# AlphacatPlus/VmambaIR

Hardware: AMD Instinct MI355X
Metric: images/sec, x4 SR 64->256 training step (fwd+bwd+Adam+EMA), full VmambaIR UNet (higher is better)
Workload: dtype bf16; 1 GPU; BASELINE.json configs[1]: x4 SR 64x64 LQ, MambaSISR6 dim48 [15,1,1,1]+15, bf16 autocast (scan arithmetic f32), batch 8 per GPU; global_batch=8, per_gpu_batch=8, parallelism=dp1, step_launch=hipGraph replay, vendor_conv_solver_search=True, vendor_conv_solver_records=bench_data/miopen, optimizer=Adam 2e-4 (0.9,0.99) + EMA 0.999, loss=L1, rccl_ranks=1, allreduce_overlapped=False, allreduce_buckets=1, allreduce_bytes=0

## Files before the change

### include/vmambair_oss.h

```cpp
#ifndef VMAMBAIR_OSS_H
#define VMAMBAIR_OSS_H

#include <stddef.h>
#include <stdint.h>

#ifdef __cplusplus
extern "C" {
#endif

#define OSS_OK 0
#define OSS_ERR_NULL (-1)
#define OSS_ERR_SHAPE (-2)
#define OSS_ERR_DSTATE (-3)
#define OSS_ERR_WORKSPACE (-4)

#define OSS_MAX_DSTATE 256

typedef enum {
    OSS_F32 = 0, OSS_F16 = 1, OSS_BF16 = 2,
    OSS_F32_BF16X3 = 3
} oss_dtype;

typedef void *oss_stream_t;

// ... 162 lines not shown
    float *zt;
    float *dts;
    float *hs;
    float *y;
    float *yc;
    float *stat;
    float *c;
    const float *pool_part;
    int n_part;
    float pool_scale;
} oss_chan_params;
int oss_chan_fwd(const oss_chan_params *p, oss_stream_t stream);
size_t oss_chan_grad_floats(int L, int dc, int Rc, int Cc);
size_t oss_chan_bwd_scratch_floats(int B, int L, int dc, int Rc, int Cc);
int oss_chan_bwd(const oss_chan_params *p, const float *gc, float *dpooled, float *grads, float *scratch, oss_stream_t stream);
int oss_rowsum(oss_dtype io, const void *a, const void *bmul, float *out, int batch, int channels, int pixels,
               int64_t a_batch_stride, int64_t a_channel_stride, int64_t b_batch_stride, int64_t b_channel_stride, float alpha,
               oss_stream_t stream);
int oss_row_affine(oss_dtype io, const void *x, const float *mul, const float *add, void *y, int batch, int channels,
                   int pixels, int64_t x_batch_stride, int64_t x_channel_stride, float alpha, oss_stream_t stream);

int oss_gelu_gate_fwd(oss_dtype io, const void *h, void *out, int batch, size_t half_elems, int64_t h_batch_stride,
                      oss_stream_t stream);
int oss_gelu_gate_bwd(oss_dtype io, const void *h, const void *dout, void *dh, int batch, size_t half_elems,
                      int64_t h_batch_stride, int64_t dout_batch_stride, oss_stream_t stream);

typedef struct {
    const void *src;
    void *dst;
    int64_t stride;
// ... 118 lines not shown
```

### vmambair_amd/csrc/oss_capi.hip

```cpp
#include <atomic>
#include <cstdlib>
#include <mutex>
#include <vector>
#include <cstring>
#include <algorithm>
#include "oss_device.h"
#include "oss_host.h"

namespace oss {

static std::atomic<int> g_force_fwd{-1}, g_force_bwd{-1};
static std::atomic<int> g_last_fwd{-1}, g_last_bwd{-1};
static std::atomic<int> g_force_fwd_seg{-1}, g_force_bwd_seg{-1};
std::atomic<int> g_last_fwd_segments{1}, g_last_bwd_segments{1}, g_last_bwd_lane_states{0};

int scan_pick_segments(long wgs, int n_chunks, int seg_req, double ovh) {
    if (seg_req == 0 || seg_req == 1 || n_chunks < 2 || wgs <= 0) return 1;
    if (seg_req > 1) return std::min(std::min(seg_req, n_chunks), kMaxSegments);
    if (wgs >= 256) return 1;
    int best = 1;
    double best_cost = (double)n_chunks;
    for (int s = 2; s <= std::min(n_chunks, 16); ++s) {
        const int cps = (n_chunks + s - 1) / s;
        if ((n_chunks + cps - 1) / cps != s) continue;
// ... 564 lines not shown
int oss_chan_fwd(const oss_chan_params *p, oss_stream_t stream) {
    fam_count(FAM_CHAN, p ? 4.0 * p->B * ((double)p->L * (2.0 * p->Cc + 2.0 * p->dc * 18.0 + 3.0) + (p->pool_part ? (double)p->n_part * p->L : p->L)) : 0.0);
    if (!p) return OSS_ERR_NULL;
    return chan_fwd(*p, reinterpret_cast<hipStream_t>(stream));
}

size_t oss_chan_grad_floats(int L, int dc, int Rc, int Cc) { return chan_grad_floats(L, dc, Rc, Cc); }
size_t oss_chan_bwd_scratch_floats(int B, int L, int dc, int Rc, int Cc) { return chan_bwd_scratch_floats(B, L, dc, Rc, Cc); }

int oss_chan_bwd(const oss_chan_params *p, const float *gc, float *dpooled, float *grads, float *scratch, oss_stream_t stream) {
    fam_count(FAM_CHAN, p ? 4.0 * p->B * ((double)p->L * (2.0 * p->Cc + 2.0 * p->dc * 18.0 + 5.0)) : 0.0);
    if (!p) return OSS_ERR_NULL;
    return chan_bwd(*p, gc, dpooled, grads, scratch, reinterpret_cast<hipStream_t>(stream));
}

int oss_rowsum(oss_dtype io, const void *a, const void *bmul, float *out, int batch, int channels, int pixels, int64_t asb,
               int64_t asc, int64_t bsb, int64_t bsc, float alpha, oss_stream_t stream) {
    if (is_f32_split(io)) return OSS_ERR_SHAPE;
    fam_count(FAM_CHAN, (double)batch * channels * pixels * esz(io) * (bmul ? 2.0 : 1.0));
    if (!a || !out) return OSS_ERR_NULL;
    if (batch <= 0 || channels <= 0 || pixels <= 0) return OSS_ERR_SHAPE;
    return rowsum(io, a, bmul, out, batch, channels, pixels, asb, asc, bsb, bsc, alpha, reinterpret_cast<hipStream_t>(stream));
}

int oss_row_affine(oss_dtype io, const void *x, const float *mul, const float *add, void *y, int batch, int channels, int pixels,
                   int64_t xsb, int64_t xsc, float alpha, oss_stream_t stream) {
    if (is_f32_split(io)) return OSS_ERR_SHAPE;
    fam_count(FAM_CHAN, (double)batch * channels * pixels * esz(io) * 2.0);
    if (!x || !y) return OSS_ERR_NULL;
    if (batch <= 0 || channels <= 0 || pixels <= 0) return OSS_ERR_SHAPE;
// ... 450 lines not shown
```

### vmambair_amd/csrc/oss_channel.hip

```cpp
#include "oss_device.h"
#include "oss_host.h"

namespace oss {

constexpr int kChN = 16;
constexpr int kChU = 8;
constexpr int kChNT = 512;
constexpr int kChRed = 8;

template <int NT>
__device__ __forceinline__ float block_sum(float v, float *red , int tid) {
    static_assert(NT == 256 || NT == 512, "block_sum: 4 or 8 waves");
    const float w = segment_sum_to_last<64>(v);
    __syncthreads();
    if ((tid & 63) == 63) red[tid >> 6] = w;
    __syncthreads();
    float t = (red[0] + red[1]) + (red[2] + red[3]);
    if constexpr (NT == 512) t += (red[4] + red[5]) + (red[6] + red[7]);
    return t;
}

__device__ __forceinline__ float sum_over_rows(float v, int lane) {
    v += __int_as_float(__builtin_amdgcn_ds_bpermute((lane ^ 16) << 2, __float_as_int(v)));
    v += __int_as_float(__builtin_amdgcn_ds_bpermute((lane ^ 32) << 2, __float_as_int(v)));
    return v;
}

template <bool use_lds, int NT>
__global__ void __launch_bounds__(NT)
oss_chan_fwd_kernel(oss_chan_params p) {
    extern __shared__ float sm[];
    const int b = blockIdx.x, tid = threadIdx.x, L = p.L, dc = p.dc, Cc = p.Cc, Rc = p.Rc;
    const bool lift = p.cin_w != nullptr;
    float *seq = sm;
    float *ybuf = seq + dc * L;
    float *ycs = ybuf + 2 * dc * L;
    float *red = ycs + L;
    float *ypart = red + kChRed;
    const bool pool_runs = p.pool_part && p.n_part >= 64;
    if (pool_runs) {
        const int ns = max(1, min(8, NT / L)), per = (p.n_part + ns - 1) / ns;
        float *run = ypart;
        for (int idx = tid; idx < ns * L; idx += NT) {
            const int sub = idx / L, l = idx - sub * L;
            const int k0 = sub * per, k1 = min(p.n_part, k0 + per);
            const float *pp = p.pool_part + (size_t)b * p.n_part * L + l;
            float sum = 0.f;
// ... 8 lines not shown
            for (; k < k1; ++k) sum += pp[(size_t)k * L];
            run[idx] = sum;
        }
        __syncthreads();
        for (int l = tid; l < L; l += NT) {
            float sum = run[l];
            for (int sub = 1; sub < ns; ++sub) sum += run[sub * L + l];
            ycs[l] = sum * p.pool_scale;
        }
        __syncthreads();
    }
    for (int l = tid; l < L; l += NT) {
        float pl;
        if (pool_runs) {
            pl = ycs[l];
            const_cast<float *>(p.pooled)[(size_t)b * L + l] = pl;
        } else if (p.pool_part) {
            const float *pp = p.pool_part + (size_t)b * p.n_part * L + l;
            float sum = 0.f;
            int k = 0;
            for (; k + 8 <= p.n_part; k += 8) {
                float v[8];
#pragma unroll
                for (int q = 0; q < 8; ++q) v[q] = pp[(size_t)(k + q) * L];
#pragma unroll
                for (int q = 0; q < 8; ++q) sum += v[q];
            }
            for (; k < p.n_part; ++k) sum += pp[(size_t)k * L];
            pl = sum * p.pool_scale;
            const_cast<float *>(p.pooled)[(size_t)b * L + l] = pl;
        } else {
            pl = p.pooled[(size_t)b * L + l];
        }
        for (int i = 0; i < dc; ++i) seq[i * L + l] = lift ? __builtin_fmaf(p.cin_w[i], pl, p.cin_b[i]) : pl;
    }
    __syncthreads();
    float *zg = p.zt + (size_t)b * 2 * L * Cc;
    float *dg = p.dts + (size_t)b * 2 * dc * L;
    float *zb, *db, *dlsF = nullptr;
    if constexpr (use_lds) { zb = ypart + 4 * 2 * dc * L; db = zb + 2 * L * Cc; dlsF = db + 2 * dc * L; } else { zb = zg; db = dg; }
    {
        const int ncol = 2 * Cc;
        const int tpc = ncol >= NT ? 1 : NT / ncol;
        for (int col = tid % (ncol < NT ? ncol : NT); col < ncol; col += NT) {
            const int sub = ncol < NT ? tid / ncol : 0;
            if (sub >= tpc) break;
            float wv[4];
#pragma unroll
            for (int i = 0; i < 4; ++i) wv[i] = i < dc ? p.Wxc[col * dc + i] : 0.f;
            const int k = col / Cc, c = col - k * Cc;
#pragma unroll 4
            for (int l = sub; l < L; l += tpc) {
                float s = 0.f;
#pragma unroll
                for (int i = 0; i < 4; ++i)
                    if (i < dc) s = __builtin_fmaf(wv[i], seq[i * L + l], s);
                zb[(k * L + l) * Cc + c] = s;
                if (use_lds) zg[(k * L + l) * Cc + c] = s;
            }
        }
    }
    __syncthreads();
    {
        const int nrow = 2 * dc, tpr = NT / nrow;
        const int row = tid / tpr, sub = tid - row * tpr;
        if (row < nrow) {
            const int k = row / dc;
            const float brow = p.dt_bias[row];
            float wr[8];
#pragma unroll
            for (int r = 0; r < 8; ++r) wr[r] = r < Rc ? p.Wdtc[row * Rc + r] : 0.f;
#pragma unroll 2
            for (int l = sub; l < L; l += tpr) {
                const float *zr = zb + (k * L + l) * Cc;
                float s = 0.f;
#pragma unroll
                for (int r = 0; r < 8; ++r)
                    if (r < Rc) s = __builtin_fmaf(wr[r], zr[r], s);
                for (int r = 8; r < Rc; ++r) s = __builtin_fmaf(p.Wdtc[row * Rc + r], zr[r], s);
                db[row * L + l] = s;
                if constexpr (use_lds) {
                    dg[row * L + l] = s;
                    float e;
                    dlsF[row * L + l] = softplus_thr(s + brow, e);
                }
            }
        }
    }
    __syncthreads();
    static_assert(NT == 512, "wave = (direction, one of four state groups)");
    constexpr int GPD = NT / 128, NPG = kChN / GPD;
    const int wave = __builtin_amdgcn_readfirstlane(tid >> 6), lane = tid & 63;
    {
        const int k = wave / GPD, ng = wave - k * GPD, n0 = ng * NPG;
        float A2[4][NPG], carry[4][NPG], Dv[4];
#pragma unroll
        for (int i = 0; i < 4; ++i) {
// ... 37 lines not shown
                        P[nn] = a0[nn] * a1[nn]; h[nn] = __builtin_fmaf(a1[nn], b0[nn], b1[nn]);
                    }
                    segment_scan4_64(P, h);
#pragma unroll
                    for (int nn = 0; nn < NPG; ++nn) {
                        const float hp = shift_from_prev_lane(h[nn], 0.f, false), Pp = shift_from_prev_lane(P[nn], 1.f, false);
                        const float hin = __builtin_fmaf(Pp, carry[i][nn], hp);
                        const float h0 = __builtin_fmaf(a0[nn], hin, b0[nn]), h1 = __builtin_fmaf(a1[nn], h0, b1[nn]);
                        hv0[nn] = h0; hv1[nn] = h1;
                        yv0[i] = __builtin_fmaf(C0[nn], h0, yv0[i]);
                        yv1[i] = __builtin_fmaf(C1[nn], h1, yv1[i]);
                        carry[i][nn] = __int_as_float(__builtin_amdgcn_readlane(__float_as_int(h1), 63));
                    }
                    float *hr = p.hs + (((size_t)b * 2 * dc + row) * L) * kChN + n0;
                    static_assert(NPG == 4, "one 16-byte store per (row, step)");
                    if (v0) *reinterpret_cast<f32x4 *>(hr + (size_t)l0 * kChN) = f32x4{hv0[0], hv0[1], hv0[2], hv0[3]};
                    if (v1) *reinterpret_cast<f32x4 *>(hr + (size_t)l1 * kChN) = f32x4{hv1[0], hv1[1], hv1[2], hv1[3]};
                    if (ng == 0) { yv0[i] = __builtin_fmaf(Dv[i], u0, yv0[i]); yv1[i] = __builtin_fmaf(Dv[i], u1, yv1[i]); }
                }
            }
#pragma unroll
            for (int i = 0; i < 4; ++i) {
                if (i < dc) {
                    float *yr = ypart + (ng * 2 * dc + k * dc + i) * L;
                    if (v0) yr[l0] = yv0[i];
                    if (v1) yr[l1] = yv1[i];
                }
            }
        }
    }
    __syncthreads();
    for (int idx = tid; idx < 2 * dc * L; idx += NT)
        ybuf[idx] = ((ypart[idx] + ypart[2 * dc * L + idx]) + ypart[2 * 2 * dc * L + idx]) + ypart[3 * 2 * dc * L + idx];
    __syncthreads();
    float part = 0.f;
    for (int l = tid; l < L; l += NT) {
        float s = lift ? p.cout_b[0] : 0.f;
        for (int i = 0; i < dc; ++i) s = __builtin_fmaf(lift ? p.cout_w[i] : 1.f, ybuf[i * L + l] + ybuf[(dc + i) * L + l], s);
        ycs[l] = s;
        part += s;
    }
    for (int idx = tid; idx < 2 * dc * L; idx += NT) p.y[(size_t)b * 2 * dc * L + idx] = ybuf[idx];
    const float mu = block_sum<NT>(part, red, tid) / (float)L;
    float q = 0.f;
    for (int l = tid; l < L; l += NT) { const float d = ycs[l] - mu; q = __builtin_fmaf(d, d, q); }
    const float rstd = 1.0f / sqrtf(block_sum<NT>(q, red, tid) / (float)L + 1e-5f);
    for (int l = tid; l < L; l += NT) {
        p.yc[(size_t)b * L + l] = ycs[l];
        p.c[(size_t)b * L + l] = __builtin_fmaf((ycs[l] - mu) * rstd, p.cn_w[l], p.cn_b[l]);
    }
    if (tid == 0) { p.stat[b * 2] = mu; p.stat[b * 2 + 1] = rstd; }
}

struct ChanSlots {
    int cnw, cnb, coutw, coutb, dA, dD, dbias, wdtc, wxc, cinw, cinb, total;
    __host__ __device__ ChanSlots(int L, int dc, int Rc, int Cc) {
        cnw = 0; cnb = L; coutw = 2 * L; coutb = coutw + dc; dA = coutb + 1; dD = dA + 2 * dc * kChN; dbias = dD + 2 * dc;
        wdtc = dbias + 2 * dc; wxc = wdtc + 2 * dc * Rc; cinw = wxc + 2 * Cc * dc; cinb = cinw + dc; total = cinb + dc;
    }
};

template <bool use_lds , int NT>
__global__ void __launch_bounds__(NT)
oss_chan_bwd_kernel(oss_chan_params p, const float *__restrict__ gc , float *__restrict__ dpool,
                    float *__restrict__ gpart, float *__restrict__ dzt, float *__restrict__ ddts, float *__restrict__ dug,
                    int stage_zdt ) {
    extern __shared__ float sm[];
    const int b = blockIdx.x, tid = threadIdx.x, L = p.L, dc = p.dc, Cc = p.Cc, Rc = p.Rc;
    const bool lift = p.cin_w != nullptr;
    const ChanSlots sl(L, dc, Rc, Cc);
    static_assert(NT == 512, "wave = (direction, one of four state groups)");
    constexpr int GPD = NT / 128, NPG = kChN / GPD;
    static_assert(NPG == 4, "16-byte accesses of a group's states");
    const int wave = __builtin_amdgcn_readfirstlane(tid >> 6), lane = tid & 63;
    const int sk = wave / GPD, sng = wave - sk * GPD, sn0 = sng * NPG;
    struct ScanOps { float B0[NPG], B1[NPG], C0[NPG], C1[NPG]; f32x4 hq0[4], hq1[4], hq2[4]; };
    auto fetch_ops = [&](int c, ScanOps &o) {
        const int u0 = c * 128 + 2 * lane;
        const int c0 = min(u0, L - 1), c1 = min(u0 + 1, L - 1), c2 = min(u0 + 2, L - 1);
        const int l0 = sk ? c0 : L - 1 - c0, l1 = sk ? c1 : L - 1 - c1, l2 = sk ? c2 : L - 1 - c2;
        const float *zsrc = p.zt + (size_t)b * 2 * L * Cc;
        const float *z0 = zsrc + (sk * L + l0) * Cc + Rc + sn0, *z1 = zsrc + (sk * L + l1) * Cc + Rc + sn0;
#pragma unroll
// ... 33 lines not shown
        for (int idx = tid; idx < 2 * dc * L; idx += NT) {
            const float x = db[idx] + p.dt_bias[idx / L];
            float e;
            dlsL[idx] = softplus_thr(x, e);
            sgsL[idx] = (x <= 20.f) ? e * __builtin_amdgcn_rcpf(1.f + e) : 1.f;
        }
    } else {
        dzb = dzt + (size_t)b * 2 * L * Cc; ddb = ddts + (size_t)b * 2 * dc * L; dub = dug + (size_t)b * 2 * dc * L;
    }
    const float mu = p.stat[b * 2], rstd = p.stat[b * 2 + 1];
    float s1 = 0.f, s2 = 0.f;
    for (int l = tid; l < L; l += NT) {
        const float pl = p.pooled[(size_t)b * L + l];
        for (int i = 0; i < dc; ++i) seq[i * L + l] = lift ? __builtin_fmaf(p.cin_w[i], pl, p.cin_b[i]) : pl;
        const float g0 = gc[(size_t)b * L + l], xh = (p.yc[(size_t)b * L + l] - mu) * rstd, g = g0 * p.cn_w[l];
        gp[sl.cnw + l] = g0 * xh;
        gp[sl.cnb + l] = g0;
        s1 += g;
        s2 = __builtin_fmaf(g, xh, s2);
    }
    const float m1 = block_sum<NT>(s1, red, tid) / (float)L;
    const float m2 = block_sum<NT>(s2, red, tid) / (float)L;
    for (int l = tid; l < L; l += NT) {
        const float xh = (p.yc[(size_t)b * L + l] - mu) * rstd, g = gc[(size_t)b * L + l] * p.cn_w[l];
        dys[l] = rstd * (g - m1 - xh * m2);
    }
    __syncthreads();
    const float *yb = p.y + (size_t)b * 2 * dc * L;
    const float *zb = p.zt + (size_t)b * 2 * L * Cc;
    {
        const int k = sk, ng = sng, n0 = sn0;
        float Av[4][NPG], carry[4][NPG], carry_a[4][NPG], accA[4][NPG], cwv[4];
// ... 81 lines not shown
            for (int i = 0; i < 4; ++i) {
                if (i < dc) {
                    const int o = (ng * 2 * dc + k * dc + i) * L;
                    if (v0) { dpl[o + l0] = ddl0[i]; dpu[o + l0] = du0[i]; }
                    if (v1) { dpl[o + l1] = ddl1[i]; dpu[o + l1] = du1[i]; }
                }
            }
            if (c + 1 < nchunk) cur = nxt;
        }
#pragma unroll
        for (int i = 0; i < 4; ++i) {
            if (i < dc) {
#pragma unroll
                for (int nn = 0; nn < NPG; ++nn) {
                    const float tA = segment_sum_to_last<64>(accA[i][nn]);
                    if (lane == 63) gp[sl.dA + (k * dc + i) * kChN + n0 + nn] = tA * Av[i][nn];
                }
            }
        }
        __syncthreads();
        if (wave < 2 * dc) {
            const int row = wave, i = row % dc;
            const float Dr = p.Dsc[row], cw = lift ? p.cout_w[i] : 1.f, bias = p.dt_bias[row];
            float sB = 0.f, sD = 0.f;
            for (int l = lane; l < L; l += 64) {
                const int o = row * L + l, st = 2 * dc * L;
                const float tl = ((dpl[o] + dpl[st + o]) + dpl[2 * st + o]) + dpl[3 * st + o];
                const float tu = ((dpu[o] + dpu[st + o]) + dpu[2 * st + o]) + dpu[3 * st + o];
                float sg;
                if constexpr (use_lds) { sg = sgsL[o]; }
                else {
                    const float x = db[o] + bias, e = exp2_hw(x * kLog2e);
                    sg = (x <= 20.f) ? e * __builtin_amdgcn_rcpf(1.f + e) : 1.f;
                }
                const float dy = cw * dys[l], ddt = tl * sg;
                ddb[o] = ddt;
                dub[o] = __builtin_fmaf(dy, Dr, tu);
                sB += ddt;
                sD = __builtin_fmaf(dy, seq[i * L + l], sD);
            }
            const float tB = segment_sum_to_last<64>(sB), tD = segment_sum_to_last<64>(sD);
            if (lane == 63) { gp[sl.dbias + row] = tB; gp[sl.dD + row] = tD; }
        }
        if (wave <= dc) {
            const int o = wave;
            float a = 0.f;
            if (lift) {
                for (int l = lane; l < L; l += 64)
                    a = o < dc ? __builtin_fmaf(dys[l], yb[o * L + l] + yb[(dc + o) * L + l], a) : a + dys[l];
            }
            const float t = segment_sum_to_last<64>(a);
            if (lane == 63) gp[sl.coutw + o] = t;
        }
    }
    __syncthreads();
    {
        const int ncol = 2 * Rc;
        const int tpc = ncol >= NT ? 1 : NT / ncol;
        for (int col = tid % (ncol < NT ? ncol : NT); col < ncol; col += NT) {
            const int sub = ncol < NT ? tid / ncol : 0;
            if (sub >= tpc) break;
            const int k = col / Rc, r = col - k * Rc;
            float wv[4];
#pragma unroll
            for (int i = 0; i < 4; ++i) wv[i] = i < dc ? p.Wdtc[(k * dc + i) * Rc + r] : 0.f;
#pragma unroll 4
            for (int l = sub; l < L; l += tpc) {
// ... 9 lines not shown
    for (int idx = tid; idx < dc * L; idx += NT) {
        const int i = idx / L, l = idx - i * L;
        float s = dub[i * L + l] + dub[(dc + i) * L + l];
        for (int k = 0; k < 2; ++k) {
            const float *dz = dzb + (k * L + l) * Cc;
            const float *wx = sWx + k * Cc * dc + i;
#pragma unroll 8
            for (int c = 0; c < Cc; ++c) s = __builtin_fmaf(wx[c * dc], dz[c], s);
        }
        dsq[idx] = s;
    }
    __syncthreads();
    for (int l = tid; l < L; l += NT) {
        float s = 0.f;
        for (int i = 0; i < dc; ++i) s = lift ? __builtin_fmaf(p.cin_w[i], dsq[i * L + l], s) : s + dsq[i * L + l];
        dpool[(size_t)b * L + l] = s;
    }
    const int n_wdtc = 2 * dc * Rc, n_wxc = 2 * Cc * dc;
    for (int o = tid; o < n_wdtc + n_wxc + 2 * dc; o += NT) {
        float s = 0.f;
        if (o < n_wdtc) {
            const int row = o / Rc, r = o - row * Rc, k = row / dc;
            if (stage_zdt) {
#pragma unroll 8
                for (int l = 0; l < L; ++l) s = __builtin_fmaf(ddb[row * L + l], zdt[(k * L + l) * Rc + r], s);
            } else {
#pragma unroll 8
                for (int l = 0; l < L; ++l) s = __builtin_fmaf(ddb[row * L + l], zb[(k * L + l) * Cc + r], s);
            }
            gp[sl.wdtc + o] = s;
        } else if (o < n_wdtc + n_wxc) {
            const int q = o - n_wdtc, i = q % dc, kc = q / dc, k = kc / Cc, c = kc - k * Cc;
#pragma unroll 8
            for (int l = 0; l < L; ++l) s = __builtin_fmaf(dzb[(k * L + l) * Cc + c], seq[i * L + l], s);
// ... 55 lines not shown
template <typename T>
__global__ void __launch_bounds__(256)
oss_row_affine_kernel(const T *__restrict__ x, const float *__restrict__ mul, const float *__restrict__ add, T *__restrict__ y,
                      int C, int P, int64_t xsb, int64_t xsc, float alpha) {
    const int row = blockIdx.y, b = row / C, c = row - b * C;
    const T *xp = x + b * xsb + c * xsc;
    T *yp = y + (size_t)row * P;
    const float *mp = mul ? mul + row : reinterpret_cast<const float *>(x), *ap = add ? add + row : mp;
    const float mv = *mp, av = *ap;
    const int p = (blockIdx.x * 256 + threadIdx.x) * 8;
    if (p >= P) return;
    const bool vec = (P % 8 == 0) && ((reinterpret_cast<uintptr_t>(xp) | reinterpret_cast<uintptr_t>(yp)) & 15u) == 0;
    float v[8];
    const int valid = min(8, P - p);
    load_items<8>(xp + p, valid, vec, v);
    const float sc = mul ? 1.f + mv : 1.f, sh = add ? alpha * av : 0.f;
#pragma unroll
    for (int i = 0; i < 8; ++i) v[i] = __builtin_fmaf(v[i], sc, sh);
    store_items<8>(yp + p, valid, vec, v);
}

size_t chan_grad_floats(int L, int dc, int Rc, int Cc) { return (size_t)ChanSlots(L, dc, Rc, Cc).total; }

constexpr size_t kChanLdsMax = 160 * 1024;
static int chan_enable_lds(const void *kern, size_t bytes) {
    if (bytes <= 48 * 1024) return 0;
    return (int)hipFuncSetAttribute(kern, hipFuncAttributeMaxDynamicSharedMemorySize, (int)kChanLdsMax);
}

static int chan_check(const oss_chan_params &p) {
    if (p.B <= 0 || p.L <= 0 || p.dc < 1 || p.dc > 4 || p.Rc < 1 || p.Cc != p.Rc + 2 * kChN) return OSS_ERR_SHAPE;
    if (!p.pooled || !p.Wxc || !p.Wdtc || !p.dt_bias || !p.A_logs || !p.Dsc || !p.cn_w || !p.cn_b || !p.zt || !p.dts || !p.hs ||
        !p.y || !p.yc || !p.stat || !p.c)
        return OSS_ERR_NULL;
    if ((p.cin_w != nullptr) != (p.cout_w != nullptr)) return OSS_ERR_NULL;
    if (p.cin_w && (!p.cin_b || !p.cout_b)) return OSS_ERR_NULL;
    return 0;
}

int chan_fwd(const oss_chan_params &p, hipStream_t s) {
    if (int e = chan_check(p)) return e;
    size_t smem = sizeof(float) * ((size_t)(3 * p.dc + 1) * p.L + kChRed + 4 * 2 * (size_t)p.dc * p.L);
    if (smem > kChanLdsMax) return OSS_ERR_SHAPE;
    const size_t extra = sizeof(float) * (2 * (size_t)p.L * p.Cc + 4 * (size_t)p.dc * p.L);
    const int use_lds = smem + extra <= kChanLdsMax ? 1 : 0;
    if (use_lds) smem += extra;
    if (use_lds) {
        if (int e = chan_enable_lds(reinterpret_cast<const void *>(oss_chan_fwd_kernel<true, kChNT>), smem)) return e;
        hipLaunchKernelGGL((oss_chan_fwd_kernel<true, kChNT>), dim3(p.B), dim3(kChNT), smem, s, p);
    } else {
        if (int e = chan_enable_lds(reinterpret_cast<const void *>(oss_chan_fwd_kernel<false, kChNT>), smem)) return e;
        hipLaunchKernelGGL((oss_chan_fwd_kernel<false, kChNT>), dim3(p.B), dim3(kChNT), smem, s, p);
    }
    return (int)hipGetLastError();
}

int chan_bwd(const oss_chan_params &p, const float *gc, float *dpool, float *gsum, float *scratch, hipStream_t s) {
    if (int e = chan_check(p)) return e;
    if (!gc || !dpool || !gsum || !scratch) return OSS_ERR_NULL;
    size_t smem = sizeof(float) * ((size_t)(2 * p.dc + 1) * p.L + kChRed + 2 * 4 * 2 * (size_t)p.dc * p.L + 2 * (size_t)p.Cc * p.dc);
    if (smem > kChanLdsMax) return OSS_ERR_SHAPE;
    const size_t zdt_bytes = sizeof(float) * 2 * (size_t)p.L * p.Rc;
    const int stage_zdt = smem + zdt_bytes <= kChanLdsMax ? 1 : 0;
    if (stage_zdt) smem += zdt_bytes;
    const size_t extra = sizeof(float) * (2 * (size_t)p.L * p.Cc + 8 * (size_t)p.dc * p.L);
    const int use_lds = smem + extra <= kChanLdsMax ? 1 : 0;
    if (use_lds) smem += extra;
    if (use_lds) {
        if (int e = chan_enable_lds(reinterpret_cast<const void *>(oss_chan_bwd_kernel<true, kChNT>), smem)) return e;
    } else {
        if (int e = chan_enable_lds(reinterpret_cast<const void *>(oss_chan_bwd_kernel<false, kChNT>), smem)) return e;
    }
    const size_t np = chan_grad_floats(p.L, p.dc, p.Rc, p.Cc);
    float *gpart = scratch;
    float *dzt = gpart + (size_t)p.B * np;
    float *ddts = dzt + (size_t)p.B * 2 * p.L * p.Cc;
    float *dug = ddts + (size_t)p.B * 2 * p.dc * p.L;
    if (use_lds) hipLaunchKernelGGL((oss_chan_bwd_kernel<true, kChNT>), dim3(p.B), dim3(kChNT), smem, s, p, gc, dpool, gpart, dzt, ddts, dug, stage_zdt);
    else         hipLaunchKernelGGL((oss_chan_bwd_kernel<false, kChNT>), dim3(p.B), dim3(kChNT), smem, s, p, gc, dpool, gpart, dzt, ddts, dug, stage_zdt);
    if (defer_finish())
        defer_sum(gpart, p.B, np, np, gsum, np, nullptr);
    else
        hipLaunchKernelGGL(oss_chan_grad_finish, dim3((unsigned)((np + 255) / 256)), dim3(256), 0, s, gpart, gsum, p.B, (int)np);
    return (int)hipGetLastError();
}

size_t chan_bwd_scratch_floats(int B, int L, int dc, int Rc, int Cc) {
    return (size_t)B * (chan_grad_floats(L, dc, Rc, Cc) + 2 * (size_t)L * Cc + 4 * (size_t)dc * L);
}

int rowsum(oss_dtype io, const void *a, const void *bmul, float *out, int B, int C, int P, int64_t asb, int64_t asc, int64_t bsb,
           int64_t bsc, float alpha, hipStream_t s) {
    dim3 grid(B * C);
// ... 24 lines not shown
```

### vmambair_amd/csrc/oss_host.h

```cpp
#pragma once
#include <hip/hip_runtime.h>
#include "../../include/vmambair_oss.h"

#include <atomic>
#include <initializer_list>

namespace oss {
struct bf16_t;
struct f16_t;

constexpr size_t kMaxLdsBytes = 160 * 1024;
struct LdsGate {
    std::atomic<size_t> enabled[16] = {};
    int ensure(const void *kern, size_t bytes) {
        if (bytes <= 48 * 1024) return 0;
        if (bytes > kMaxLdsBytes) return OSS_ERR_SHAPE;
        int dev = 0;
        (void)hipGetDevice(&dev);
        std::atomic<size_t> &slot = enabled[dev & 15];
        if (bytes <= slot.load(std::memory_order_acquire)) return 0;
        const hipError_t e = hipFuncSetAttribute(kern, hipFuncAttributeMaxDynamicSharedMemorySize, (int)bytes);
        if (e != hipSuccess) return (int)e;
        size_t cur = slot.load(std::memory_order_relaxed);
        while (cur < bytes && !slot.compare_exchange_weak(cur, bytes, std::memory_order_release)) {}
// ... 105 lines not shown
int conv1x1_wgrad(oss_dtype io, const void *dy, const void *x, float *dw, float *part, int B, int M, int N, int P,
                  int64_t gsb, int64_t gsm, int64_t xsb, int64_t xsn, hipStream_t s, int G = 1, int64_t gsg = 0, int64_t xsg = 0,
                  int Mh = 0, int64_t gs_hi = 0, float *db = nullptr, int f32_split = 0);
int proj_fwd(oss_dtype io, const void *x2, const float *Wx, const float *Wdt, void *xdbl, void *dts, int B, int D, int C, int R,
             int L, hipStream_t s, int f32_split = 0);
int proj_dgrad(oss_dtype io, const void *ddts, void *dxdbl, const void *du, const float *Wx, const float *Wdt, void *dx2, int B,
               int D, int C, int R, int L, hipStream_t s, int f32_split = 0);
void proj_force_valu(int on);
bool proj_mfma_ok(oss_dtype io, int B, int D, int C, int R, int L);
int cross_scan2(oss_dtype it, oss_dtype ot, const void *x, void *x2, int B, int D, int H, int W, int64_t xsb, int64_t xsc,
                hipStream_t s);
int cross_merge2(oss_dtype io, const void *g2, void *dx, int B, int D, int H, int W, hipStream_t s);
size_t chan_grad_floats(int L, int dc, int Rc, int Cc);
size_t chan_bwd_scratch_floats(int B, int L, int dc, int Rc, int Cc);
int chan_fwd(const oss_chan_params &p, hipStream_t s);
int chan_bwd(const oss_chan_params &p, const float *gc, float *dpool, float *gsum, float *scratch, hipStream_t s);
int rowsum(oss_dtype io, const void *a, const void *bmul, float *out, int B, int C, int P, int64_t asb, int64_t asc, int64_t bsb,
           int64_t bsc, float alpha, hipStream_t s);
int row_affine(oss_dtype io, const void *x, const float *mul, const float *add, void *y, int B, int C, int P, int64_t xsb,
               int64_t xsc, float alpha, hipStream_t s);
int gelu_gate_fwd(oss_dtype io, const void *h, void *out, int B, size_t n, int64_t hsb, hipStream_t s);
int gelu_gate_bwd(oss_dtype io, const void *h, const void *dout, void *dh, int B, size_t n, int64_t hsb, int64_t gsb, hipStream_t s);
bool defer_wgrad();
void defer_wgrad_push(const void *desc, size_t bytes, unsigned blocks);
size_t wgrad_desc_bytes();
int wgrad_grouped_launch(int io, const void *d_descs, const void *d_map, unsigned total_blocks, hipStream_t s);
void wgrad_desc_set_first_block(void *desc, unsigned first);
int wgrad_desc_io(const void *desc);
bool defer_finish();
void defer_sum(const float *src, int K, size_t stride, size_t V, float *dst0, size_t n0, float *dst1);
int sum_partials_multi(const oss_sum_chunk *chunks, int n_chunks, hipStream_t s);
// ... 9 lines not shown
```

### vmambair_amd/ops/channel.py

```python
from __future__ import annotations

import contextlib
import os
from typing import List, Optional

import torch

from .. import _capi
from ._common import (_DT, _LIB, _check, _f32c, _fork_for_wgrad, _keep, _keep_views, _planes, _ptr)


def chan_supported(dc: int, n_state: int, d_inner: int) -> bool:
    lds_bwd = 4 * ((18 * dc + 1) * d_inner + 2 * dc * (dc + 32 + 8) + 8)
    return n_state == 16 and 1 <= dc <= 4 and lds_bwd <= 160 * 1024


def _chan_params(B, L, pooled, prm, saved, c):
    cin_w, cin_b, Wxc, Wdtc, dt_bias, A_logs, Dsc, cout_w, cout_b, cn_w, cn_b = prm
    zt, dts, hs, y, yc, stat = saved
    P = _capi.ChanParams()
    P.B, P.L, P.dc, P.Rc, P.Cc = B, L, Wdtc.shape[1], Wdtc.shape[2], Wxc.shape[1]
    for name, t in (("pooled", pooled), ("cin_w", cin_w), ("cin_b", cin_b), ("Wxc", Wxc), ("Wdtc", Wdtc), ("dt_bias", dt_bias),
                    ("A_logs", A_logs), ("Dsc", Dsc), ("cout_w", cout_w), ("cout_b", cout_b), ("cn_w", cn_w), ("cn_b", cn_b),
                    ("zt", zt), ("dts", dts), ("hs", hs), ("y", y), ("yc", yc), ("stat", stat), ("c", c)):
        setattr(P, name, _ptr(t))
    P.pool_part, P.n_part, P.pool_scale = None, 0, 0.0
    return P


# ... 15 lines not shown
             torch.empty((B, 2 * dc, d), **f), torch.empty((B, d), **f), torch.empty((B, 2), **f))
    out = torch.empty((B, d, H, W), dtype=y2.dtype, device=dev)
    if y2.numel() == 0:
        return [out, c, pooled, *saved]
    lib = _capi.load()
    with torch.cuda.device(dev):
        st = torch.cuda.current_stream().cuda_stream
        P = _chan_params(B, d, pooled, prm, saved, c)
        if pool_part is not None and pool_part.numel():
            _check(pool_part.dtype == torch.float32 and pool_part.is_contiguous() and pool_part.dim() == 3 and
                   pool_part.shape[0] == B and pool_part.shape[2] == d, "chan_gate: pool_part must be contiguous (B, tiles, d) float32")
            P.pool_part, P.n_part, P.pool_scale = pool_part.data_ptr(), pool_part.shape[1], 1.0 / (H * W)
        else:
            _capi.check(lib.oss_rowsum(_DT[y2.dtype], y2.data_ptr(), None, pooled.data_ptr(), B, d, H * W, y2.stride(0), y2.stride(1),
                                       0, 0, 1.0 / (H * W), st), "oss_rowsum")
        _capi.check(lib.oss_chan_fwd(P, st), "oss_chan_fwd")
        _capi.check(lib.oss_row_affine(_DT[y2.dtype], y2.data_ptr(), c.data_ptr() if mul_mode else None,
                                       None if mul_mode else c.data_ptr(), out.data_ptr(), B, d, H * W, y2.stride(0),
                                       y2.stride(1), 1.0, st), "oss_row_affine")
    return [out, c, pooled, *saved]


def chan_gate_bwd(g: torch.Tensor, y2: torch.Tensor, c: torch.Tensor, pooled: torch.Tensor, zt: torch.Tensor, dts: torch.Tensor,
                  hs: torch.Tensor, y: torch.Tensor, yc: torch.Tensor, stat: torch.Tensor, cin_w: Optional[torch.Tensor],
                  cin_b: Optional[torch.Tensor], Wxc: torch.Tensor, Wdtc: torch.Tensor, dt_bias: torch.Tensor,
                  A_logs: torch.Tensor, Dsc: torch.Tensor, cout_w: Optional[torch.Tensor], cout_b: Optional[torch.Tensor],
                  cn_w: torch.Tensor, cn_b: torch.Tensor, mul_mode: bool, fold: bool = False) -> List[torch.Tensor]:
    B, d, H, W = y2.shape
    y2, g = _planes(y2), _planes(g)
    if g.dtype != y2.dtype:
        g = g.to(y2.dtype)
    prm = tuple(_f32c(t) for t in (cin_w, cin_b, Wxc, Wdtc, dt_bias, A_logs, Dsc, cout_w, cout_b, cn_w, cn_b))
    dc, Rc, Cc = Wdtc.shape[1], Wdtc.shape[2], Wxc.shape[1]
    dev = y2.device
    lib = _capi.load()
    f = dict(dtype=torch.float32, device=dev)
    gc, dpool = torch.empty((B, d), **f), torch.empty((B, d), **f)
    grads = torch.empty((int(lib.oss_chan_grad_floats(d, dc, Rc, Cc)),), **f)
    scratch = torch.empty((int(lib.oss_chan_bwd_scratch_floats(B, d, dc, Rc, Cc)),), **f)
    dy2 = None if fold else torch.empty((B, d, H, W), dtype=y2.dtype, device=dev)
    with torch.cuda.device(dev):
        st = torch.cuda.current_stream().cuda_stream
        _capi.check(lib.oss_rowsum(_DT[y2.dtype], g.data_ptr(), y2.data_ptr() if mul_mode else None, gc.data_ptr(), B, d, H * W,
                                   g.stride(0), g.stride(1), y2.stride(0), y2.stride(1), 1.0, st), "oss_rowsum")
        _capi.check(lib.oss_chan_bwd(_chan_params(B, d, pooled, prm, (zt, dts, hs, y, yc, stat), c), gc.data_ptr(),
                                     dpool.data_ptr(), grads.data_ptr(), scratch.data_ptr(), st), "oss_chan_bwd")
        _keep(scratch, grads)
        if fold:
            return [dpool, grads]
        _capi.check(lib.oss_row_affine(_DT[y2.dtype], g.data_ptr(), c.data_ptr() if mul_mode else None, dpool.data_ptr(),
                                       dy2.data_ptr(), B, d, H * W, g.stride(0), g.stride(1), 1.0 / (H * W), st), "oss_row_affine")
    return [dy2, grads]


_CH = "Tensor? cin_w, Tensor? cin_b, Tensor Wxc, Tensor Wdtc, Tensor dt_bias, Tensor A_logs, Tensor Dsc, Tensor? cout_w, " \
      "Tensor? cout_b, Tensor cn_w, Tensor cn_b, bool mul_mode"
_LIB.define(f"chan_gate_fwd(Tensor y2, {_CH}, Tensor? pool_part=None) -> Tensor[]")
_LIB.define(f"chan_gate_bwd(Tensor g, Tensor y2, Tensor c, Tensor pooled, Tensor zt, Tensor dts, Tensor hs, Tensor y, Tensor yc, "
            f"Tensor stat, {_CH}, bool fold=False) -> Tensor[]")
_LIB.impl("chan_gate_fwd", chan_gate_fwd, "CUDA")
_LIB.impl("chan_gate_bwd", chan_gate_bwd, "CUDA")
# ... 88 lines not shown
```

Before: 244.5 images/s.

## Fuse channel-gate affine into chan fwd kernel and slice bwd weight sums across CUs

The channel-attention forward kernel now also applies the gate affine to the feature map. Its grid is widened to (B, slices), and each slice gates a range of pixels. Every slice recomputes the small channel SSM redundantly, and only slice 0 writes the saved tensors. The backward kernel similarly gets a y-grid dimension that splits the weight-gradient reduction slots across blocks, again recomputing the per-batch prologue. The aim is to remove a separate row_affine launch and to raise occupancy when B=8 leaves most CUs idle, at the cost of duplicated SSM work per slice.

```diff
diff --git a/include/vmambair_oss.h b/include/vmambair_oss.h
--- a/include/vmambair_oss.h
+++ b/include/vmambair_oss.h
@@ -200,6 +200,13 @@
 size_t oss_chan_grad_floats(int L, int dc, int Rc, int Cc);
 size_t oss_chan_bwd_scratch_floats(int B, int L, int dc, int Rc, int Cc);
 int oss_chan_bwd(const oss_chan_params *p, const float *gc, float *dpooled, float *grads, float *scratch, oss_stream_t stream);
+int oss_chan_gate_fwd_ok(int L, int dc, int Rc, int Cc);
+int oss_chan_gate_slices(int batch, int pixels, int compute_units);
+int oss_chan_gate_fwd(const oss_chan_params *p, oss_dtype io, const void *y2, int64_t y2_batch_stride, int64_t y2_channel_stride,
+                      void *out, int pixels, int mul_add, int slices, oss_stream_t stream);
+int oss_chan_bwd_slices(int batch, int L, int dc, int Rc, int Cc, int compute_units);
+int oss_chan_bwd_sliced(const oss_chan_params *p, const float *gc, float *dpooled, float *grads, float *scratch, int slices,
+                        oss_stream_t stream);
 int oss_rowsum(oss_dtype io, const void *a, const void *bmul, float *out, int batch, int channels, int pixels,
                int64_t a_batch_stride, int64_t a_channel_stride, int64_t b_batch_stride, int64_t b_channel_stride, float alpha,
                oss_stream_t stream);
diff --git a/vmambair_amd/csrc/oss_capi.hip b/vmambair_amd/csrc/oss_capi.hip
--- a/vmambair_amd/csrc/oss_capi.hip
+++ b/vmambair_amd/csrc/oss_capi.hip
@@ -602,6 +602,30 @@
     return chan_bwd(*p, gc, dpooled, grads, scratch, reinterpret_cast<hipStream_t>(stream));
 }
 
+int oss_chan_gate_fwd_ok(int L, int dc, int Rc, int Cc) { return chan_gate_fwd_ok(L, dc, Rc, Cc); }
+int oss_chan_gate_slices(int batch, int pixels, int compute_units) { return chan_gate_slices(batch, pixels, compute_units); }
+
+int oss_chan_gate_fwd(const oss_chan_params *p, oss_dtype io, const void *y2, int64_t y2_batch_stride, int64_t y2_channel_stride,
+                      void *out, int pixels, int mul_add, int slices, oss_stream_t stream) {
+    if (is_f32_split(io)) return OSS_ERR_SHAPE;
+    fam_count(FAM_CHAN, p ? 4.0 * p->B * ((double)p->L * (2.0 * p->Cc + 2.0 * p->dc * 18.0 + 3.0) + (p->pool_part ? (double)p->n_part * p->L : p->L)) +
+                              (double)p->B * p->L * (pixels > 0 ? pixels : 0) * esz(io) * 2.0 : 0.0);
+    if (!p) return OSS_ERR_NULL;
+    return chan_gate_fwd(*p, io, y2, y2_batch_stride, y2_channel_stride, out, pixels, mul_add, slices, reinterpret_cast<hipStream_t>(stream));
+}
+
+int oss_chan_bwd_slices(int batch, int L, int dc, int Rc, int Cc, int compute_units) {
+    return chan_bwd_slices(batch, L, dc, Rc, Cc, compute_units);
+}
+
+int oss_chan_bwd_sliced(const oss_chan_params *p, const float *gc, float *dpooled, float *grads, float *scratch, int slices,
+                        oss_stream_t stream) {
+    fam_count(FAM_CHAN, p ? 4.0 * p->B * ((double)p->L * (2.0 * p->Cc + 2.0 * p->dc * 18.0 + 5.0)) : 0.0);
+    if (!p) return OSS_ERR_NULL;
+    if (slices < 0) return OSS_ERR_SHAPE;
+    return chan_bwd(*p, gc, dpooled, grads, scratch, reinterpret_cast<hipStream_t>(stream), slices);
+}
+
 int oss_rowsum(oss_dtype io, const void *a, const void *bmul, float *out, int batch, int channels, int pixels, int64_t asb,
                int64_t asc, int64_t bsb, int64_t bsc, float alpha, oss_stream_t stream) {
     if (is_f32_split(io)) return OSS_ERR_SHAPE;
diff --git a/vmambair_amd/csrc/oss_channel.hip b/vmambair_amd/csrc/oss_channel.hip
--- a/vmambair_amd/csrc/oss_channel.hip
+++ b/vmambair_amd/csrc/oss_channel.hip
@@ -1,5 +1,7 @@
 #include "oss_device.h"
 #include "oss_host.h"
+
+#include <type_traits>
 
 namespace oss {
 
@@ -26,11 +28,72 @@
     return v;
 }
 
-template <bool use_lds, int NT>
+template <int I>
+__device__ __forceinline__ void affine_items(float (&v)[I], float sc, float sh) {
+#pragma unroll
+    for (int i = 0; i < I; ++i) {
+        v[i] = __builtin_fmaf(v[i], sc, sh);
+        asm volatile("" : "+v"(v[i]));
+    }
+}
+
+struct ChanGate {
+    const void *y2;
+    void *out;
+    int64_t ysb, ysc;
+    int P, io, mul;
+    int per;
+};
+struct ChanNoGate {};
+
+constexpr int kGateU = 4;
+
+template <typename T, int NT>
+__device__ __forceinline__ void chan_gate_slice(const ChanGate &g, const float *cs , int b, int L, int slice, int nslice,
+                                                int tid) {
+    const int p0 = slice * g.per, p1 = slice == nslice - 1 ? g.P : p0 + g.per;
+    const int nv = (p1 - p0 + 7) >> 3;
+    const T *x = reinterpret_cast<const T *>(g.y2) + b * g.ysb;
+    T *y = reinterpret_cast<T *>(g.out) + (size_t)b * L * g.P;
+    const bool mul = g.mul != 0;
+    constexpr int U = kGateU;
+    const int total = L * nv;
+    for (int base = tid; base < total; base += NT * U) {
+        float v[U][8];
+        const T *xp[U];
+        T *yp[U];
+        int valid[U], row[U];
+        bool vec[U];
+#pragma unroll
+        for (int u = 0; u < U; ++u) {
+            const int idx = min(base + u * NT, total - 1);
+            const int l = idx / nv, p = p0 + 8 * (idx - l * nv);
+            row[u] = l;
+            xp[u] = x + l * g.ysc + p;
+            yp[u] = y + (size_t)l * g.P + p;
+            valid[u] = min(8, p1 - p);
+            vec[u] = valid[u] == 8 && ((reinterpret_cast<uintptr_t>(xp[u]) | reinterpret_cast<uintptr_t>(yp[u])) & 15u) == 0;
+            load_items<8>(xp[u], valid[u], vec[u], v[u]);
+        }
+#pragma unroll
+        for (int u = 0; u < U; ++u) {
+            if (base + u * NT < total) {
+                const float cv = cs[row[u]];
+                affine_items<8>(v[u], mul ? 1.f + cv : 1.f, mul ? 0.f : cv);
+                store_items<8>(yp[u], valid[u], vec[u], v[u]);
+            }
+        }
+    }
+}
+
+template <bool use_lds, int NT, typename Gate = ChanNoGate>
 __global__ void __launch_bounds__(NT)
-oss_chan_fwd_kernel(oss_chan_params p) {
+oss_chan_fwd_kernel(oss_chan_params p, Gate gate) {
     extern __shared__ float sm[];
+    constexpr bool GATE = !std::is_same<Gate, ChanNoGate>::value;
+    static_assert(!GATE || use_lds, "the gated launch exists in the LDS form only");
     const int b = blockIdx.x, tid = threadIdx.x, L = p.L, dc = p.dc, Cc = p.Cc, Rc = p.Rc;
+    const bool w0 = !GATE || blockIdx.y == 0;
     const bool lift = p.cin_w != nullptr;
     float *seq = sm;
     float *ybuf = seq + dc * L;
@@ -69,7 +132,7 @@
         float pl;
         if (pool_runs) {
             pl = ycs[l];
-            const_cast<float *>(p.pooled)[(size_t)b * L + l] = pl;
+            if (w0) const_cast<float *>(p.pooled)[(size_t)b * L + l] = pl;
         } else if (p.pool_part) {
             const float *pp = p.pool_part + (size_t)b * p.n_part * L + l;
             float sum = 0.f;
@@ -83,7 +146,7 @@
             }
             for (; k < p.n_part; ++k) sum += pp[(size_t)k * L];
             pl = sum * p.pool_scale;
-            const_cast<float *>(p.pooled)[(size_t)b * L + l] = pl;
+            if (w0) const_cast<float *>(p.pooled)[(size_t)b * L + l] = pl;
         } else {
             pl = p.pooled[(size_t)b * L + l];
         }
@@ -111,7 +174,7 @@
                 for (int i = 0; i < 4; ++i)
                     if (i < dc) s = __builtin_fmaf(wv[i], seq[i * L + l], s);
                 zb[(k * L + l) * Cc + c] = s;
-                if (use_lds) zg[(k * L + l) * Cc + c] = s;
+                if (use_lds && w0) zg[(k * L + l) * Cc + c] = s;
             }
         }
     }
@@ -135,7 +198,7 @@
                 for (int r = 8; r < Rc; ++r) s = __builtin_fmaf(p.Wdtc[row * Rc + r], zr[r], s);
                 db[row * L + l] = s;
                 if constexpr (use_lds) {
-                    dg[row * L + l] = s;
+                    if (w0) dg[row * L + l] = s;
                     float e;
                     dlsF[row * L + l] = softplus_thr(s + brow, e);
                 }
@@ -203,8 +266,8 @@
                     }
                     float *hr = p.hs + (((size_t)b * 2 * dc + row) * L) * kChN + n0;
                     static_assert(NPG == 4, "one 16-byte store per (row, step)");
-                    if (v0) *reinterpret_cast<f32x4 *>(hr + (size_t)l0 * kChN) = f32x4{hv0[0], hv0[1], hv0[2], hv0[3]};
-                    if (v1) *reinterpret_cast<f32x4 *>(hr + (size_t)l1 * kChN) = f32x4{hv1[0], hv1[1], hv1[2], hv1[3]};
+                    if (v0 && w0) *reinterpret_cast<f32x4 *>(hr + (size_t)l0 * kChN) = f32x4{hv0[0], hv0[1], hv0[2], hv0[3]};
+                    if (v1 && w0) *reinterpret_cast<f32x4 *>(hr + (size_t)l1 * kChN) = f32x4{hv1[0], hv1[1], hv1[2], hv1[3]};
                     if (ng == 0) { yv0[i] = __builtin_fmaf(Dv[i], u0, yv0[i]); yv1[i] = __builtin_fmaf(Dv[i], u1, yv1[i]); }
                 }
             }
@@ -229,16 +292,27 @@
         ycs[l] = s;
         part += s;
     }
-    for (int idx = tid; idx < 2 * dc * L; idx += NT) p.y[(size_t)b * 2 * dc * L + idx] = ybuf[idx];
+    if (w0)
+        for (int idx = tid; idx < 2 * dc * L; idx += NT) p.y[(size_t)b * 2 * dc * L + idx] = ybuf[idx];
     const float mu = block_sum<NT>(part, red, tid) / (float)L;
     float q = 0.f;
     for (int l = tid; l < L; l += NT) { const float d = ycs[l] - mu; q = __builtin_fmaf(d, d, q); }
     const float rstd = 1.0f / sqrtf(block_sum<NT>(q, red, tid) / (float)L + 1e-5f);
     for (int l = tid; l < L; l += NT) {
-        p.yc[(size_t)b * L + l] = ycs[l];
-        p.c[(size_t)b * L + l] = __builtin_fmaf((ycs[l] - mu) * rstd, p.cn_w[l], p.cn_b[l]);
-    }
-    if (tid == 0) { p.stat[b * 2] = mu; p.stat[b * 2 + 1] = rstd; }
+        const float cv = __builtin_fmaf((ycs[l] - mu) * rstd, p.cn_w[l], p.cn_b[l]);
+        if (w0) { p.yc[(size_t)b * L + l] = ycs[l]; p.c[(size_t)b * L + l] = cv; }
+        if constexpr (GATE) ycs[l] = cv;
+    }
+    if (tid == 0 && w0) { p.stat[b * 2] = mu; p.stat[b * 2 + 1] = rstd; }
+    if constexpr (GATE) {
+        __syncthreads();
+        const int slice = blockIdx.y, nslice = gridDim.y;
+        switch (gate.io) {
+            case OSS_F32: chan_gate_slice<float, NT>(gate, ycs, b, L, slice, nslice, tid); break;
+            case OSS_F16: chan_gate_slice<f16_t, NT>(gate, ycs, b, L, slice, nslice, tid); break;
+            default: chan_gate_slice<bf16_t, NT>(gate, ycs, b, L, slice, nslice, tid); break;
+        }
+    }
 }
 
 struct ChanSlots {
@@ -249,13 +323,15 @@
     }
 };
 
-template <bool use_lds , int NT>
+template <bool use_lds , int NT, bool SLICED = false>
 __global__ void __launch_bounds__(NT)
 oss_chan_bwd_kernel(oss_chan_params p, const float *__restrict__ gc , float *__restrict__ dpool,
                     float *__restrict__ gpart, float *__restrict__ dzt, float *__restrict__ ddts, float *__restrict__ dug,
                     int stage_zdt ) {
     extern __shared__ float sm[];
+    static_assert(!SLICED || use_lds, "the sliced launch exists in the LDS form only");
     const int b = blockIdx.x, tid = threadIdx.x, L = p.L, dc = p.dc, Cc = p.Cc, Rc = p.Rc;
+    const bool w0 = !SLICED || blockIdx.y == 0;
     const bool lift = p.cin_w != nullptr;
     const ChanSlots sl(L, dc, Rc, Cc);
     static_assert(NT == 512, "wave = (direction, one of four state groups)");
@@ -319,8 +395,7 @@
         const float pl = p.pooled[(size_t)b * L + l];
         for (int i = 0; i < dc; ++i) seq[i * L + l] = lift ? __builtin_fmaf(p.cin_w[i], pl, p.cin_b[i]) : pl;
         const float g0 = gc[(size_t)b * L + l], xh = (p.yc[(size_t)b * L + l] - mu) * rstd, g = g0 * p.cn_w[l];
-        gp[sl.cnw + l] = g0 * xh;
-        gp[sl.cnb + l] = g0;
+        if (w0) { gp[sl.cnw + l] = g0 * xh; gp[sl.cnb + l] = g0; }
         s1 += g;
         s2 = __builtin_fmaf(g, xh, s2);
     }
@@ -432,7 +507,7 @@
 #pragma unroll
                 for (int nn = 0; nn < NPG; ++nn) {
                     const float tA = segment_sum_to_last<64>(accA[i][nn]);
-                    if (lane == 63) gp[sl.dA + (k * dc + i) * kChN + n0 + nn] = tA * Av[i][nn];
+                    if (lane == 63 && w0) gp[sl.dA + (k * dc + i) * kChN + n0 + nn] = tA * Av[i][nn];
                 }
             }
         }
@@ -458,7 +533,7 @@
                 sD = __builtin_fmaf(dy, seq[i * L + l], sD);
             }
             const float tB = segment_sum_to_last<64>(sB), tD = segment_sum_to_last<64>(sD);
-            if (lane == 63) { gp[sl.dbias + row] = tB; gp[sl.dD + row] = tD; }
+            if (lane == 63 && w0) { gp[sl.dbias + row] = tB; gp[sl.dD + row] = tD; }
         }
         if (wave <= dc) {
             const int o = wave;
@@ -468,7 +543,7 @@
                     a = o < dc ? __builtin_fmaf(dys[l], yb[o * L + l] + yb[(dc + o) * L + l], a) : a + dys[l];
             }
             const float t = segment_sum_to_last<64>(a);
-            if (lane == 63) gp[sl.coutw + o] = t;
+            if (lane == 63 && w0) gp[sl.coutw + o] = t;
         }
     }
     __syncthreads();
@@ -508,10 +583,12 @@
     for (int l = tid; l < L; l += NT) {
         float s = 0.f;
         for (int i = 0; i < dc; ++i) s = lift ? __builtin_fmaf(p.cin_w[i], dsq[i * L + l], s) : s + dsq[i * L + l];
-        dpool[(size_t)b * L + l] = s;
-    }
-    const int n_wdtc = 2 * dc * Rc, n_wxc = 2 * Cc * dc;
-    for (int o = tid; o < n_wdtc + n_wxc + 2 * dc; o += NT) {
+        if (w0) dpool[(size_t)b * L + l] = s;
+    }
+    const int n_wdtc = 2 * dc * Rc, n_wxc = 2 * Cc * dc, n_slot = n_wdtc + n_wxc + 2 * dc;
+    const int per_slice = SLICED ? (n_slot + (int)gridDim.y - 1) / (int)gridDim.y : n_slot;
+    const int o_begin = SLICED ? (int)blockIdx.y * per_slice : 0, o_end = min(n_slot, o_begin + per_slice);
+    for (int o = o_begin + tid; o < o_end; o += NT) {
         float s = 0.f;
         if (o < n_wdtc) {
             const int row = o / Rc, r = o - row * Rc, k = row / dc;
@@ -597,9 +674,7 @@
     float v[8];
     const int valid = min(8, P - p);
     load_items<8>(xp + p, valid, vec, v);
-    const float sc = mul ? 1.f + mv : 1.f, sh = add ? alpha * av : 0.f;
-#pragma unroll
-    for (int i = 0; i < 8; ++i) v[i] = __builtin_fmaf(v[i], sc, sh);
+    affine_items<8>(v, mul ? 1.f + mv : 1.f, add ? alpha * av : 0.f);
     store_items<8>(yp + p, valid, vec, v);
 }
 
@@ -621,26 +696,81 @@
     return 0;
 }
 
+static size_t chan_fwd_lds(int L, int dc, int Cc, int &use_lds) {
+    size_t smem = sizeof(float) * ((size_t)(3 * dc + 1) * L + kChRed + 4 * 2 * (size_t)dc * L);
+    const size_t extra = sizeof(float) * (2 * (size_t)L * Cc + 4 * (size_t)dc * L);
+    use_lds = smem + extra <= kChanLdsMax ? 1 : 0;
+    return use_lds ? smem + extra : smem;
+}
+
+static int chan_compute_units() {
+    static const int n = [] {
+        int dev = 0, cus = 0;
+        if (hipGetDevice(&dev) != hipSuccess) return 0;
+        if (hipDeviceGetAttribute(&cus, hipDeviceAttributeMultiprocessorCount, dev) != hipSuccess) return 0;
+        return cus;
+    }();
+    return n;
+}
+
+int chan_gate_fwd_ok(int L, int dc, int Rc, int Cc) {
+    if (L <= 0 || dc < 1 || dc > 4 || Rc < 1 || Cc != Rc + 2 * kChN) return 0;
+    int use_lds;
+    (void)chan_fwd_lds(L, dc, Cc, use_lds);
+    return use_lds;
+}
+
+int chan_gate_slices(int B, int P, int cus) {
+    if (cus <= 0) cus = chan_compute_units();
+    if (B <= 0 || P <= 0) return 1;
+    return max(1, min(cus / B, P / 8));
+}
+
+int chan_gate_fwd(const oss_chan_params &p, oss_dtype io, const void *y2, int64_t ysb, int64_t ysc, void *out, int P, int mul,
+                  int slices, hipStream_t s) {
+    if (int e = chan_check(p)) return e;
+    if (!y2 || !out) return OSS_ERR_NULL;
+    if (P <= 0 || slices < 0 || (io != OSS_F32 && io != OSS_F16 && io != OSS_BF16) || !chan_gate_fwd_ok(p.L, p.dc, p.Rc, p.Cc))
+        return OSS_ERR_SHAPE;
+    int use_lds;
+    const size_t smem = chan_fwd_lds(p.L, p.dc, p.Cc, use_lds);
+    const int S = slices ? max(1, min(min(slices, P / 8), 65535)) : min(chan_gate_slices(p.B, P, 0), 65535);
+    ChanGate g;
+    g.y2 = y2; g.out = out; g.ysb = ysb; g.ysc = ysc; g.P = P; g.io = (int)io; g.mul = mul ? 1 : 0;
+    g.per = (P / S) & ~7;
+    auto kern = oss_chan_fwd_kernel<true, kChNT, ChanGate>;
+    if (int e = chan_enable_lds(reinterpret_cast<const void *>(kern), smem)) return e;
+    hipLaunchKernelGGL(kern, dim3(p.B, S), dim3(kChNT), smem, s, p, g);
+    return (int)hipGetLastError();
+}
+
 int chan_fwd(const oss_chan_params &p, hipStream_t s) {
     if (int e = chan_check(p)) return e;
-    size_t smem = sizeof(float) * ((size_t)(3 * p.dc + 1) * p.L + kChRed + 4 * 2 * (size_t)p.dc * p.L);
+    int use_lds;
+    const size_t smem = chan_fwd_lds(p.L, p.dc, p.Cc, use_lds);
     if (smem > kChanLdsMax) return OSS_ERR_SHAPE;
-    const size_t extra = sizeof(float) * (2 * (size_t)p.L * p.Cc + 4 * (size_t)p.dc * p.L);
-    const int use_lds = smem + extra <= kChanLdsMax ? 1 : 0;
-    if (use_lds) smem += extra;
     if (use_lds) {
         if (int e = chan_enable_lds(reinterpret_cast<const void *>(oss_chan_fwd_kernel<true, kChNT>), smem)) return e;
-        hipLaunchKernelGGL((oss_chan_fwd_kernel<true, kChNT>), dim3(p.B), dim3(kChNT), smem, s, p);
+        hipLaunchKernelGGL((oss_chan_fwd_kernel<true, kChNT>), dim3(p.B), dim3(kChNT), smem, s, p, ChanNoGate{});
     } else {
         if (int e = chan_enable_lds(reinterpret_cast<const void *>(oss_chan_fwd_kernel<false, kChNT>), smem)) return e;
-        hipLaunchKernelGGL((oss_chan_fwd_kernel<false, kChNT>), dim3(p.B), dim3(kChNT), smem, s, p);
+        hipLaunchKernelGGL((oss_chan_fwd_kernel<false, kChNT>), dim3(p.B), dim3(kChNT), smem, s, p, ChanNoGate{});
     }
     return (int)hipGetLastError();
 }
 
-int chan_bwd(const oss_chan_params &p, const float *gc, float *dpool, float *gsum, float *scratch, hipStream_t s) {
+int chan_bwd_slices(int B, int L, int dc, int Rc, int Cc, int cus) {
+    (void)L;
+    if (cus <= 0) cus = chan_compute_units();
+    if (B <= 0 || dc < 1 || Rc < 1 || Cc < 1) return 1;
+    const int n_slot = 2 * dc * Rc + 2 * Cc * dc + 2 * dc;
+    return max(1, min(cus / B, (n_slot + 63) / 64));
+}
+
+int chan_bwd(const oss_chan_params &p, const float *gc, float *dpool, float *gsum, float *scratch, hipStream_t s, int slices) {
     if (int e = chan_check(p)) return e;
     if (!gc || !dpool || !gsum || !scratch) return OSS_ERR_NULL;
+    if (slices < -1) return OSS_ERR_SHAPE;
     size_t smem = sizeof(float) * ((size_t)(2 * p.dc + 1) * p.L + kChRed + 2 * 4 * 2 * (size_t)p.dc * p.L + 2 * (size_t)p.Cc * p.dc);
     if (smem > kChanLdsMax) return OSS_ERR_SHAPE;
     const size_t zdt_bytes = sizeof(float) * 2 * (size_t)p.L * p.Rc;
@@ -649,7 +779,10 @@
     const size_t extra = sizeof(float) * (2 * (size_t)p.L * p.Cc + 8 * (size_t)p.dc * p.L);
     const int use_lds = smem + extra <= kChanLdsMax ? 1 : 0;
     if (use_lds) smem += extra;
-    if (use_lds) {
+    const bool sliced = use_lds && slices >= 0;
+    if (sliced) {
+        if (int e = chan_enable_lds(reinterpret_cast<const void *>(oss_chan_bwd_kernel<true, kChNT, true>), smem)) return e;
+    } else if (use_lds) {
         if (int e = chan_enable_lds(reinterpret_cast<const void *>(oss_chan_bwd_kernel<true, kChNT>), smem)) return e;
     } else {
         if (int e = chan_enable_lds(reinterpret_cast<const void *>(oss_chan_bwd_kernel<false, kChNT>), smem)) return e;
@@ -659,7 +792,11 @@
     float *dzt = gpart + (size_t)p.B * np;
     float *ddts = dzt + (size_t)p.B * 2 * p.L * p.Cc;
     float *dug = ddts + (size_t)p.B * 2 * p.dc * p.L;
-    if (use_lds) hipLaunchKernelGGL((oss_chan_bwd_kernel<true, kChNT>), dim3(p.B), dim3(kChNT), smem, s, p, gc, dpool, gpart, dzt, ddts, dug, stage_zdt);
+    if (sliced) {
+        const int n_slot = 2 * p.dc * p.Rc + 2 * p.Cc * p.dc + 2 * p.dc;
+        const int S = slices ? min(slices, n_slot) : chan_bwd_slices(p.B, p.L, p.dc, p.Rc, p.Cc, 0);
+        hipLaunchKernelGGL((oss_chan_bwd_kernel<true, kChNT, true>), dim3(p.B, S), dim3(kChNT), smem, s, p, gc, dpool, gpart, dzt, ddts, dug, stage_zdt);
+    } else if (use_lds) hipLaunchKernelGGL((oss_chan_bwd_kernel<true, kChNT>), dim3(p.B), dim3(kChNT), smem, s, p, gc, dpool, gpart, dzt, ddts, dug, stage_zdt);
     else         hipLaunchKernelGGL((oss_chan_bwd_kernel<false, kChNT>), dim3(p.B), dim3(kChNT), smem, s, p, gc, dpool, gpart, dzt, ddts, dug, stage_zdt);
     if (defer_finish())
         defer_sum(gpart, p.B, np, np, gsum, np, nullptr);
diff --git a/vmambair_amd/csrc/oss_host.h b/vmambair_amd/csrc/oss_host.h
--- a/vmambair_amd/csrc/oss_host.h
+++ b/vmambair_amd/csrc/oss_host.h
@@ -143,7 +143,12 @@
 size_t chan_grad_floats(int L, int dc, int Rc, int Cc);
 size_t chan_bwd_scratch_floats(int B, int L, int dc, int Rc, int Cc);
 int chan_fwd(const oss_chan_params &p, hipStream_t s);
-int chan_bwd(const oss_chan_params &p, const float *gc, float *dpool, float *gsum, float *scratch, hipStream_t s);
+int chan_bwd(const oss_chan_params &p, const float *gc, float *dpool, float *gsum, float *scratch, hipStream_t s, int slices = -1);
+int chan_gate_fwd_ok(int L, int dc, int Rc, int Cc);
+int chan_gate_slices(int B, int P, int cus);
+int chan_gate_fwd(const oss_chan_params &p, oss_dtype io, const void *y2, int64_t ysb, int64_t ysc, void *out, int P, int mul,
+                  int slices, hipStream_t s);
+int chan_bwd_slices(int B, int L, int dc, int Rc, int Cc, int cus);
 int rowsum(oss_dtype io, const void *a, const void *bmul, float *out, int B, int C, int P, int64_t asb, int64_t asc, int64_t bsb,
            int64_t bsc, float alpha, hipStream_t s);
 int row_affine(oss_dtype io, const void *x, const float *mul, const float *add, void *y, int B, int C, int P, int64_t xsb,
diff --git a/vmambair_amd/ops/channel.py b/vmambair_amd/ops/channel.py
--- a/vmambair_amd/ops/channel.py
+++ b/vmambair_amd/ops/channel.py
@@ -13,6 +13,11 @@
 def chan_supported(dc: int, n_state: int, d_inner: int) -> bool:
     lds_bwd = 4 * ((18 * dc + 1) * d_inner + 2 * dc * (dc + 32 + 8) + 8)
     return n_state == 16 and 1 <= dc <= 4 and lds_bwd <= 160 * 1024
+
+
+_CGF = os.environ.get("VMAMBAIR_CHAN_GATE_FUSED", "1")
+CHAN_GATE_FUSED = {"fwd", "sums"} if _CGF == "1" else set() if _CGF == "0" else set(_CGF.split(","))
+GATE_SLICES = 0
 
 
 def _chan_params(B, L, pooled, prm, saved, c):
@@ -58,6 +63,10 @@
         else:
             _capi.check(lib.oss_rowsum(_DT[y2.dtype], y2.data_ptr(), None, pooled.data_ptr(), B, d, H * W, y2.stride(0), y2.stride(1),
                                        0, 0, 1.0 / (H * W), st), "oss_rowsum")
+        if "fwd" in CHAN_GATE_FUSED and lib.oss_chan_gate_fwd_ok(d, dc, Rc, Cc):
+            _capi.check(lib.oss_chan_gate_fwd(P, _DT[y2.dtype], y2.data_ptr(), y2.stride(0), y2.stride(1), out.data_ptr(), H * W,
+                                              1 if mul_mode else 0, GATE_SLICES, st), "oss_chan_gate_fwd")
+            return [out, c, pooled, *saved]
         _capi.check(lib.oss_chan_fwd(P, st), "oss_chan_fwd")
         _capi.check(lib.oss_row_affine(_DT[y2.dtype], y2.data_ptr(), c.data_ptr() if mul_mode else None,
                                        None if mul_mode else c.data_ptr(), out.data_ptr(), B, d, H * W, y2.stride(0),
@@ -87,8 +96,12 @@
         st = torch.cuda.current_stream().cuda_stream
         _capi.check(lib.oss_rowsum(_DT[y2.dtype], g.data_ptr(), y2.data_ptr() if mul_mode else None, gc.data_ptr(), B, d, H * W,
                                    g.stride(0), g.stride(1), y2.stride(0), y2.stride(1), 1.0, st), "oss_rowsum")
-        _capi.check(lib.oss_chan_bwd(_chan_params(B, d, pooled, prm, (zt, dts, hs, y, yc, stat), c), gc.data_ptr(),
-                                     dpool.data_ptr(), grads.data_ptr(), scratch.data_ptr(), st), "oss_chan_bwd")
+        P = _chan_params(B, d, pooled, prm, (zt, dts, hs, y, yc, stat), c)
+        if "sums" in CHAN_GATE_FUSED:
+            _capi.check(lib.oss_chan_bwd_sliced(P, gc.data_ptr(), dpool.data_ptr(), grads.data_ptr(), scratch.data_ptr(), GATE_SLICES,
+                                                st), "oss_chan_bwd_sliced")
+        else:
+            _capi.check(lib.oss_chan_bwd(P, gc.data_ptr(), dpool.data_ptr(), grads.data_ptr(), scratch.data_ptr(), st), "oss_chan_bwd")
         _keep(scratch, grads)
         if fold:
             return [dpool, grads]
```

Result: no change. 245.2 images/s, median of 6 (+0.3%).
